# KDL-umass/CausalGPSLC.jl

Hardware: AMD Instinct MI355X
Metric: posterior samples/sec (kernel+chol+predict) at N=4096; SATE rel-err vs CPU (higher is better)
Workload: dtype f64; 1 GPU; Synthetic N=4096 D=8 nU=2, unit A (Gram build + potrf + alpha + MeanITE + SATE mean/var), L=1 level(s), 1024 posterior samples per GPU per step; levels=1, mean_ite=True

## Files before the change

### causalgpslc.jl_amd/csrc/back_block.h

```cpp
#pragma once
#include "gpslc_internal.h"

__device__ __forceinline__ void tile_tv32(const double* __restrict__ t, const double* v ,
                                          int wave, int lane, double out[32]) {
    const double v0 = v[lane], v1 = v[lane + 64];
    double p[32];
#pragma unroll
    for (int cc = 0; cc < 32; ++cc) {
        const double* col = t + (wave * 32 + cc) * GP_TS;
        p[cc] = col[lane] * v0 + col[lane + 64] * v1;
    }
#pragma unroll
    for (int cc = 0; cc < 32; ++cc) {
        double x = p[cc];
#pragma unroll
        for (int o = 32; o >= 1; o >>= 1) x += __shfl_xor(x, o, 64);
        out[cc] = x;
    }
}

__device__ __forceinline__ void tile_tv16_issue(const double* __restrict__ t, int wave, int half, int lane, double (&raw)[32]) {
#pragma unroll
    for (int cc = 0; cc < 16; ++cc) {
        const double* col = t + (wave * 32 + half * 16 + cc) * GP_TS;
        raw[cc] = __builtin_nontemporal_load(col + lane);
        raw[16 + cc] = __builtin_nontemporal_load(col + lane + 64);
    }
}
__device__ __forceinline__ double tile_tv16_finish(const double (&raw)[32], const double* v , int lane) {
    const double v0 = v[lane], v1 = v[lane + 64];
    double p[16], q8[8], q4[4], q2[2];
#pragma unroll
    for (int cc = 0; cc < 16; ++cc) p[cc] = raw[cc] * v0 + raw[16 + cc] * v1;
    const bool b5 = (lane & 32) != 0, b4 = (lane & 16) != 0, b3 = (lane & 8) != 0, b2 = (lane & 4) != 0;
#pragma unroll
    for (int j = 0; j < 8; ++j) {
        const double send = b5 ? p[j] : p[8 + j], keep = b5 ? p[8 + j] : p[j];
        q8[j] = keep + __shfl_xor(send, 32, 64);
    }
#pragma unroll
    for (int j = 0; j < 4; ++j) {
        const double send = b4 ? q8[j] : q8[4 + j], keep = b4 ? q8[4 + j] : q8[j];
        q4[j] = keep + __shfl_xor(send, 16, 64);
    }
#pragma unroll
    for (int j = 0; j < 2; ++j) {
        const double send = b3 ? q4[j] : q4[2 + j], keep = b3 ? q4[2 + j] : q4[j];
        q2[j] = keep + __shfl_xor(send, 8, 64);
    }
    const double send = b2 ? q2[0] : q2[1], keep = b2 ? q2[1] : q2[0];
    double x = keep + __shfl_xor(send, 4, 64);
    x += __shfl_xor(x, 2, 64);
    x += __shfl_xor(x, 1, 64);
    return x;
}

__device__ __forceinline__ void back_task_body(const TRef& M, const TRef& F, const int b, const int nt, double* __restrict__ alpha_out,
                                               double* lds, const int tid) {
    double* z = lds;
    double* al = lds + nt * GP_TS;
    const int lane = tid & 63;
    const int wave = __builtin_amdgcn_readfirstlane(tid >> 6);
    const int col = wave * 32 + (lane >> 2);
    const bool writer = (lane & 3) == 0;
    double ra[32], rb[32];
    tile_tv16_issue(tref_tile(F, b, 0, nt - 1), wave, 0, lane, ra);
    tile_tv16_issue(tref_tile(F, b, 0, nt - 1), wave, 1, lane, rb);
    for (int e = tid; e < nt * GP_TS; e += 256) z[e] = tref_tile(M, b, nt, e >> 7)[(e & 127) * GP_TS];
    __syncthreads();
    for (int i = nt - 1; i >= 0; --i) {
        {
            const double* nxt = i > 0 ? tref_tile(M, b, i, i - 1) : nullptr;
            const double m0 = tile_tv16_finish(ra, z + i * GP_TS, lane);
            if (nxt) tile_tv16_issue(nxt, wave, 0, lane, ra);
            const double m1 = tile_tv16_finish(rb, z + i * GP_TS, lane);
            if (nxt) tile_tv16_issue(nxt, wave, 1, lane, rb);
            if (writer) {
                al[i * GP_TS + col] = m0;
                al[i * GP_TS + col + 16] = m1;
                alpha_out[i * GP_TS + col] = m0;
                alpha_out[i * GP_TS + col + 16] = m1;
            }
        }
        __syncthreads();
        for (int k = i - 1; k >= 0; --k) {
            const double* nxt = k > 0 ? tref_tile(M, b, i, k - 1) : tref_tile(F, b, 0, i - 1);
            const double m0 = tile_tv16_finish(ra, al + i * GP_TS, lane);
            tile_tv16_issue(nxt, wave, 0, lane, ra);
            const double m1 = tile_tv16_finish(rb, al + i * GP_TS, lane);
            tile_tv16_issue(nxt, wave, 1, lane, rb);
            if (writer) {
                z[k * GP_TS + col] -= m0;
                z[k * GP_TS + col + 16] -= m1;
            }
        }
        __syncthreads();
    }
}
```

### causalgpslc.jl_amd/csrc/gpslc_internal.h

```cpp
#pragma once
#include <hip/hip_runtime.h>
#include <stdint.h>

#define GP_TS 128
#define GP_TSQ (GP_TS * GP_TS)

typedef double d4 __attribute__((ext_vector_type(4)));
typedef double d2 __attribute__((ext_vector_type(2)));

#define MAXF 32

#include <atomic>
#include <cstdlib>
struct DeviceOnce {
    std::atomic<unsigned long long> mask{0};
};
inline void lds_opt_in(DeviceOnce& o, const void* fn, int bytes) {
    int dev = 0;
    (void)hipGetDevice(&dev);
    const unsigned long long bit = 1ull << (dev & 63);
    if (o.mask.load(std::memory_order_acquire) & bit) return;
    (void)hipFuncSetAttribute(fn, hipFuncAttributeMaxDynamicSharedMemorySize, bytes);
    o.mask.fetch_or(bit, std::memory_order_release);
}
inline int device_cus() {
    static std::atomic<int> cus[64];
    int dev = 0;
    (void)hipGetDevice(&dev);
    int v = cus[dev & 63].load(std::memory_order_relaxed);
    if (v == 0) {
        v = 256;
        (void)hipDeviceGetAttribute(&v, hipDeviceAttributeMultiprocessorCount, dev);
        cus[dev & 63].store(v, std::memory_order_relaxed);
    }
    return v;
}
inline int diag_env(const char* name, int dflt) {
#ifdef GPSLC_DIAG
    const char* e = getenv(name);
    return e ? atoi(e) : dflt;
#else
    (void)name;
    return dflt;
#endif
}

struct TRef {
    double* base;
    long long bstride;
    int kind;
    int ro, co;
    int ld;
    int bdiv;
};

__host__ __device__ inline long long tref_index(const TRef& t, int i, int j) {
    long long ii = (long long)i + t.ro, jj = (long long)j + t.co;
    return t.kind == 0 ? ii * (ii + 1) / 2 + jj : ii * (long long)t.ld + jj;
}
__host__ __device__ inline double* tref_tile(const TRef& t, long long b, int i, int j) {
    if (t.bdiv > 1) b /= t.bdiv;
    return t.base + b * t.bstride + tref_index(t, i, j) * (long long)GP_TSQ;
}

struct GemmArgs {
    TRef A, B, C;
    int shape;
    int i0, j0;
    int mi, mj;
    int k0, k1;
    int accumulate;
    int nbatch;
    int ntiles;
    int short_row0;
    int short_rows;
    int sym;
    int fuse;
    TRef F;
    int fk;
    int skip_gdiag;
    int* info;
    int info_base;
    int* queue;
    const unsigned short* order;
    int diag_skip;
    unsigned long long* dbg;
};

struct SampleParams {
    const double* U;
    const double* uyLS;
    const double* xyLS;
    const double* tyLS;
    const double* yScale;
    const double* yNoise;
    long long u_sstride;
};

struct SampleGrid {
    const double* X;
    const double* T;
    SampleParams p;
    long long s0;
    int n, nX, nU, nt;
    __host__ __device__ const double* column(long long s, int f) const {
        return f < nU ? p.U + s * p.u_sstride + (long long)f * n : X + (long long)(f - nU) * n;
    }
    __host__ __device__ double lengthscale(long long s, int f) const {
        return f < nU ? p.uyLS[s * nU + f] : p.xyLS[s * nX + (f - nU)];
    }
};

struct GramArgs : SampleGrid {
    TRef M;
    double* part;
    int with_sums;
    int f32;
    int binary_t;
    unsigned long long* dbg;
};

#include "task_list.h"
struct PotrfTaskArgs {
    GemmArgs g;
    const unsigned* list;
    int* sync;
    int* timeout;
    int nt;
    double* alpha;
    int fence_mode;
    unsigned long long* dbg;
};
void launch_potrf_tasks(const PotrfTaskArgs& a, long long ntasks, int mt, hipStream_t st);

void launch_tile_gemm(const GemmArgs& g, hipStream_t st);
void launch_syrk_diag(const GemmArgs& g, int carry_aug, hipStream_t st);
void launch_diag_update_potrf(const GemmArgs& g, int carry_aug, hipStream_t st);
void launch_diag(const TRef& M, int k, double* inv, long long inv_bstride, int* info,
                 int info_base, int nbatch, hipStream_t st);
void launch_gram(const GramArgs& g, int nbatch, hipStream_t st);
void launch_diag_robust(const TRef& M, int k, int* info, int info_base, int nbatch, hipStream_t st);
void launch_trsm_robust(const TRef& X, const TRef& L, int k, int i0, int count, int nbatch, hipStream_t st);
void launch_fold_pair_info(const int* pair_info, int* info, int gs, int lc, hipStream_t st);

struct RhsArgs {
    const double* T; const double* Y; const double* tyLS; const double* doT;
    long long y_sstride;
    long long s0; int n, nt, naug, L; int with_sums;
    const double* part; double* bsum; double* ksum; double* sumdelta;
    TRef M;
    int live_rows;
    const double* doT_base;
    const double* W; int G;
    const double* bw; const double* kw; double* wnorm2;
};
void launch_rhs(const RhsArgs& r, int nbatch, hipStream_t st);

struct WsumArgs : SampleGrid {
    int G;
    const double* W;
    double* bw; double* kw;
    int with_k;
    int binary_t;
};
void launch_wsum(const WsumArgs& a, int nbatch, hipStream_t st);

struct EpiArgs {
    TRef M; int n, nt, naug, L; long long s0; long long S;
    const double* sumdelta; double pred_noise;
    double* meanSATE; double* varSATE;
    double* logdet; double* quad;
    int from_rows;
    const double* wnorm2; int wL;
};
void launch_epilogue(const EpiArgs& e, int nbatch, hipStream_t st);

struct BackArgs {
    TRef M; const double* inv; long long inv_bstride; int nt; int naug;
    double* zwork;
};
void launch_backsolve(const BackArgs& a, int nbatch, hipStream_t st);

struct IteMeanArgs : SampleGrid {
    long long S;
    int L; const double* doT;
    const double* alpha;
    const double* Y;
    long long y_sstride;
    const double* yNoise;
    double* meanITE;
    long long si, ss, sl;
    int f32;
    const double* doT_base;
};
void launch_ite_mean(const IteMeanArgs& a, int nbatch, hipStream_t st);

struct VecArgs : SampleGrid {
    int L;
    const double* doT;
    TRef M; double* part; double* sumdelta;
    const double* alpha; const double* Y; long long y_sstride;
    double* meanITE; long long si, ss, sl;
};
void launch_vec_sums(const VecArgs& a, int nbatch, hipStream_t st);
void launch_vec_mean(const VecArgs& a, int nbatch, hipStream_t st);

void launch_rbf_log(const double* X1, const double* X2, long long n, int d, const double* ls,
                    int ls_len, double* out, hipStream_t st);
void launch_process_cov(const double* in, long long n, double scale, double noise, double* out,
                        hipStream_t st);

struct DtArgs : SampleGrid {
    const double* doT;
    int l0, lc;
    int vec;
// ... 80 lines not shown
```

### causalgpslc.jl_amd/csrc/k_tilegemm.hip

```cpp
#include "gpslc_internal.h"
#include "diag_block.h"
#include "back_block.h"

#ifdef GPSLC_DIAG
#define GP_DBG_ON(g) ((g).dbg != nullptr)
#define GP_DIAG_SKIP(g) ((g).diag_skip)
#define GP_FENCE_MODE(a) ((a).fence_mode & 1)
#define GP_TASK_PRIO(a) (((a).fence_mode >> 4) & 3)
#define GP_TASK_WITHHOLD(a, b, is_diag, k) ((((a).fence_mode >> 6) & 1) && (b) == 0 && (is_diag) && (k) == 1)
#else
#define GP_DBG_ON(g) false
#define GP_DIAG_SKIP(g) 0
#define GP_FENCE_MODE(a) 0
#define GP_TASK_PRIO(a) 3
#define GP_TASK_WITHHOLD(a, b, is_diag, k) false
#endif

#define KLOOP_BARRIER asm volatile("s_waitcnt lgkmcnt(0)\n\ts_barrier" ::: "memory")
#define MFMA_PRIO_UP __builtin_amdgcn_s_setprio(1)
#define MFMA_PRIO_DOWN __builtin_amdgcn_s_setprio(0)

#define KS 16
#define LROW 144
#define OPER_LDS (KS * LROW)
// ... 140 lines not shown
                    xb[u] = *reinterpret_cast<const d2*>(pb + (tid + 256 * u) * 2);
                }
            };
            auto lstore = [&](int buf, const d2 (&xa)[4], const d2 (&xb)[4]) {
#pragma unroll
                for (int u = 0; u < 4; ++u) {
                    *reinterpret_cast<d2*>(lA + buf * OPER_LDS + loff[u]) = xa[u];
                    *reinterpret_cast<d2*>(lB + buf * OPER_LDS + loff[u]) = xb[u];
                }
            };
            auto compute = [&](int buf, int s) {
                const double* pa = lA + buf * OPER_LDS + frow_a;
                const double* pb = lB + buf * OPER_LDS + frow_b;
                const int nlo = ACC ? 0 : min(4, max(0, (s & 7) - 4 * wc));
                constexpr bool PIPE = ACC && DIAG == 0;
                double afn[4], bfn[4];
                if (PIPE) {
#pragma unroll
                    for (int m = 0; m < 4; ++m) afn[m] = pa[16 * m];
#pragma unroll
                    for (int n = 0; n < 4; ++n) bfn[n] = pb[16 * n];
                }
#pragma unroll
                for (int ks = 0; ks < KS / 4; ++ks) {
                    double af[4], bf[4];
                    if (PIPE) {
#pragma unroll
                        for (int m = 0; m < 4; ++m) { af[m] = afn[m]; bf[m] = bfn[m]; }
                        if (ks + 1 < KS / 4) {
#pragma unroll
                            for (int m = 0; m < 4; ++m) afn[m] = pa[(ks + 1) * 4 * LROW + 16 * m];
#pragma unroll
                            for (int n = 0; n < 4; ++n) bfn[n] = pb[(ks + 1) * 4 * LROW + 16 * n];
                        }
                    } else {
#pragma unroll
                        for (int m = 0; m < 4; ++m) af[m] = pa[ks * 4 * LROW + 16 * m];
#pragma unroll
                        for (int n = 0; n < 4; ++n) bf[n] = pb[ks * 4 * LROW + 16 * n];
                    }
                    if (mlive == 4 && nlo == 0) {
#pragma unroll
                        for (int m = 0; m < 4; ++m)
#pragma unroll
                            for (int n = 0; n < 4; ++n)
                                acc[m][n] = mfma_step<ACC>(bf[n], af[m], acc[m][n]);
                    } else {
#pragma unroll
                        for (int m = 0; m < 4; ++m)
                            if (m < mlive) {
#pragma unroll
                                for (int n = 0; n < 4; ++n)
                                    if (n >= nlo) acc[m][n] = mfma_step<ACC>(bf[n], af[m], acc[m][n]);
                            }
                    }
                }
            };

            auto compute_p = [&](int buf, int s) {
                const int sl = s & 7;
                if (sl > 7 - pw) return;
                const bool use0 = sl <= pw;
                const double* pa = lA + buf * OPER_LDS + (lane >> 4) * LROW + (lane & 15);
                const double* pb = lB + buf * OPER_LDS + (lane >> 4) * LROW + (lane & 15);
#pragma unroll
                for (int ks = 0; ks < KS / 4; ++ks) {
                    const double b0 = pb[ks * 4 * LROW + 16 * pw];
                    const double b1 = pb[ks * 4 * LROW + 16 * (7 - pw)];
                    double af[8];
#pragma unroll
                    for (int m = 0; m < 8; ++m) af[m] = pa[ks * 4 * LROW + 16 * m];
#pragma unroll
                    for (int m = 0; m < 8; ++m)
                        if (m < prow) {
                            if (use0) acc[m >> 1][2 * (m & 1)] = mfma_step<0>(b0, af[m], acc[m >> 1][2 * (m & 1)]);
                            acc[m >> 1][2 * (m & 1) + 1] = mfma_step<0>(b1, af[m], acc[m >> 1][2 * (m & 1) + 1]);
                        }
                }
            };

            gload(0, ra, rb);
            lstore(0, ra, rb);
            gload(1, ra, rb);
            __syncthreads();
            if (GP_DBG_ON(g)) st1 = __builtin_amdgcn_s_memtime();
            if (DIAG == 0) {
                for (int s = 0; s < nslab; s += 2) {
                    if (s + 2 < nslab) gload(s + 2, ra2, rb2);
                    MFMA_PRIO_UP;
                    if (ACC) compute(0, s); else compute_p(0, s);
                    MFMA_PRIO_DOWN;
                    lstore(1, ra, rb);
                    KLOOP_BARRIER;
                    if (s + 3 < nslab) gload(s + 3, ra, rb);
                    MFMA_PRIO_UP;
                    if (ACC) compute(1, s + 1); else compute_p(1, s + 1);
                    MFMA_PRIO_DOWN;
                    if (s + 2 < nslab) lstore(0, ra2, rb2);
                    KLOOP_BARRIER;
                }
            } else {
                for (int s = 0; s < nslab; s += 2) {
                    compute(0, s);
                    if (DIAG == 1) lstore(1, ra, rb);
                    __syncthreads();
                    compute(1, s + 1);
                    if (DIAG == 1) lstore(0, ra, rb);
                    __syncthreads();
                }
            }
        }
        if (GP_DBG_ON(g)) st2 = __builtin_amdgcn_s_memtime();

        {
        if (!ACC) {
            double* __restrict__ Cp = Ct + ((lane >> 4) * GP_TS + (lane & 15));
#pragma unroll
            for (int m = 0; m < 8; ++m)
                if (m < prow) {
#pragma unroll
                    for (int v = 0; v < 4; ++v) {
                        Cp[(16 * pw + 4 * v) * GP_TS + 16 * m] = acc[m >> 1][2 * (m & 1)][v];
                        Cp[(16 * (7 - pw) + 4 * v) * GP_TS + 16 * m] = acc[m >> 1][2 * (m & 1) + 1][v];
                    }
                }
        } else {
            int soff = ccol * GP_TS + crow;
            asm volatile("" : "+v"(soff));
            double* __restrict__ Cs = Ct + soff;
#pragma unroll
            for (int n = 0; n < 4; ++n)
#pragma unroll
                for (int v = 0; v < 4; ++v)
#pragma unroll
                    for (int m = 0; m < 4; ++m)
                        Cs[(16 * n + 4 * v) * GP_TS + 16 * m] = acc[m][n][v];
        }
        }
        if (GP_DBG_ON(g)) {
            asm volatile("s_waitcnt vmcnt(0)" ::: "memory");
            const unsigned long long st3 = __builtin_amdgcn_s_memtime();
            if (tid == 0) {
                unsigned long long* d = g.dbg + (size_t)item * 8;
                d[0] = st0; d[1] = st1; d[2] = st2; d[3] = st3;
                d[4] = __builtin_amdgcn_s_getreg((31 << 11) | 4);
                d[5] = __builtin_amdgcn_s_getreg((31 << 11) | 20);
                d[6] = __builtin_amdgcn_s_memrealtime();
                d[7] = blockIdx.x;
            }
        }
    });
}

typedef const __attribute__((address_space(1))) char* gcptr;
__device__ __forceinline__ gcptr wave_uniform(const void* p) {
    const unsigned long long x = (unsigned long long)p;
    const unsigned lo = __builtin_amdgcn_readfirstlane((unsigned)x);
    const unsigned hi = __builtin_amdgcn_readfirstlane((unsigned)(x >> 32));
    return (gcptr)(((unsigned long long)hi << 32) | lo);
}
typedef unsigned u4 __attribute__((ext_vector_type(4)));
template <bool WT>
__device__ __forceinline__ void strip_store2(__amdgpu_buffer_rsrc_t rs, double* tile_lane, int lane_bytes, int col_doubles, d2 v) {
    if (WT) __builtin_amdgcn_raw_buffer_store_b128(__builtin_bit_cast(u4, v), rs, lane_bytes + col_doubles * 8, 0,  16);
    else __builtin_nontemporal_store(v, reinterpret_cast<d2*>(tile_lane + col_doubles));
}

template <int WD, bool AUGEP = false, bool WT = false>
__device__ __forceinline__ void strip_item(const GemmArgs& g, const int b, const int ti, const int tj, const bool no_update,
                                           const int nslab, double* lB, const int tid, const int lane,
                                           const int wave, const int li, const int lg, const int frow_b,
                                           const int (&loff)[4], const long long item, const bool with_aug = false) {
    double* __restrict__ Ct = tref_tile(g.C, b, ti, tj);
    const bool live = !(g.short_rows > 0 && ti >= g.short_row0 && 32 * wave >= g.short_rows);
    unsigned long long st0 = 0, st1 = 0, st2 = 0;
    if (GP_DBG_ON(g)) st0 = __builtin_amdgcn_s_memtime();
    const int lane_off = lg * GP_TS + 32 * wave + 2 * li;

    d4 acc[2][8];
    if (live) {
        const double* __restrict__ Cl = Ct + lane_off;
#pragma unroll
        for (int n = 0; n < 8; ++n)
#pragma unroll
            for (int v = 0; v < 4; ++v) {
                const d2 c = __builtin_nontemporal_load(reinterpret_cast<const d2*>(Cl + (16 * n + 4 * v) * GP_TS));
                acc[0][n][v] = c[0];
                acc[1][n][v] = c[1];
            }
    }

    if (nslab > 0 && !no_update) {
        constexpr int SLAB = KS * GP_TS * 8;
        const int nsl = __builtin_amdgcn_readfirstlane(nslab);
        const __amdgpu_buffer_rsrc_t rA = __builtin_amdgcn_make_buffer_rsrc(
            (void*)(unsigned long long)wave_uniform(tref_tile(g.A, b, ti, g.k0)), 0, nsl * SLAB, 0x00020000);
        const __amdgpu_buffer_rsrc_t rB = __builtin_amdgcn_make_buffer_rsrc(
            (void*)(unsigned long long)wave_uniform(tref_tile(g.B, b, tj, g.k0)), 0, nsl * SLAB, 0x00020000);
        int voa[4], vob[4];
#pragma unroll
        for (int u = 0; u < 4; ++u) {
            voa[u] = (4 * u * GP_TS + lane_off) * 8;
            vob[u] = (tid + 256 * u) * 16;
        }
        const std::true_type yes;
        const std::false_type no;
        auto kloop = [&](auto lv) {
            constexpr bool LIVE = decltype(lv)::value;
            d2 rb[4], rb2[4];
            d2 a0[4], a1[4];
            auto bload1 = [&](int so, int u) { return __builtin_bit_cast(d2, __builtin_amdgcn_raw_buffer_load_b128(rB, vob[u], so, 0)); };
            auto bload = [&](int so, d2 (&xb)[4]) {
#pragma unroll
                for (int u = 0; u < 4; ++u) xb[u] = bload1(so, u);
            };
            auto aload = [&](int so, int ks) {
                return __builtin_bit_cast(d2, __builtin_amdgcn_raw_buffer_load_b128(rA, voa[ks], so,  2));
            };
            auto lstore = [&](int buf, const d2 (&xb)[4]) {
#pragma unroll
                for (int u = 0; u < 4; ++u) *reinterpret_cast<d2*>(lB + buf * OPER_LDS + loff[u]) = xb[u];
            };
            auto slab = [&](auto pf, int buf, d2 (&aa)[4], int so, d2 (&lb)[4], auto ws, int wbuf,
                            const d2 (&wb)[4]) {
                constexpr bool PF = decltype(pf)::value;
                constexpr bool WS = decltype(ws)::value;
                const double* pb = lB + buf * OPER_LDS + frow_b;
#pragma unroll
                for (int ks = 0; ks < KS / 4; ++ks) {
                    if (LIVE) {
                        double bf[8];
#pragma unroll
                        for (int n = 0; n < 8; ++n) bf[n] = pb[ks * 4 * LROW + 16 * n];
                        const d2 a = aa[ks];
#pragma unroll
                        for (int n = 0; n < 8; ++n)
#pragma unroll
                            for (int m = 0; m < 2; ++m) acc[m][n] = mfma_step<1>(bf[n], a[m], acc[m][n]);
                        if (PF) aa[ks] = aload(so, ks);
                    }
                    if (PF) lb[ks] = bload1(so, ks);
                    if (WS) *reinterpret_cast<d2*>(lB + wbuf * OPER_LDS + loff[ks]) = wb[ks];
                }
            };
            bload(0, rb);
            if (LIVE) {
#pragma unroll
                for (int ks = 0; ks < 4; ++ks) a0[ks] = aload(0, ks);
#pragma unroll
                for (int ks = 0; ks < 4; ++ks) a1[ks] = aload(SLAB, ks);
            }
            lstore(0, rb);
            bload(SLAB, rb);
            KLOOP_BARRIER;
            if (GP_DBG_ON(g)) st1 = __builtin_amdgcn_s_memtime();
            int so = 2 * SLAB;
            for (int s = 0; s + 2 < nsl; s += 2) {
                slab(yes, 0, a0, so, rb2, yes, 1, rb);
                KLOOP_BARRIER;
                slab(yes, 1, a1, so + SLAB, rb, yes, 0, rb2);
                KLOOP_BARRIER;
                so += 2 * SLAB;
            }
            slab(no, 0, a0, 0, rb2, yes, 1, rb);
            KLOOP_BARRIER;
            slab(no, 1, a1, 0, rb, no, 0, rb2);
            KLOOP_BARRIER;
        };
        if (live) kloop(yes); else kloop(no);
    }
    if (GP_DBG_ON(g)) st2 = __builtin_amdgcn_s_memtime();

    if (live) {
        const double* __restrict__ Wl = tref_tile(g.F, b, 0, g.fk) + (lg * GP_TS + li);
        double* __restrict__ Co = Ct + lane_off;
        const __amdgpu_buffer_rsrc_t crs = __builtin_amdgcn_make_buffer_rsrc((void*)(unsigned long long)wave_uniform(Ct), 0, GP_TSQ * 8, 0x00020000);
        double wn[WD];
        int pc = 0, pn = 0, pv = 0;
#pragma unroll
        for (int q = 0; q < WD; ++q) {
            wn[q] = Wl[(16 * pn + 4 * pv) * GP_TS + 16 * pc];
            if (++pv == 4) { pv = 0; if (++pn > pc) { pn = 0; ++pc; } }
        }
        int q = 0;
#pragma unroll
        for (int nc = 0; nc < 8; ++nc) {
            d4 st[2];
            st[0] = (d4){0.0, 0.0, 0.0, 0.0};
            st[1] = (d4){0.0, 0.0, 0.0, 0.0};
#pragma unroll
            for (int n = 0; n < 8; ++n)
                if (n <= nc) {
#pragma unroll
                    for (int v = 0; v < 4; ++v) {
                        const double w = wn[q % WD];
                        if (pc < 8) {
                            wn[q % WD] = Wl[(16 * pn + 4 * pv) * GP_TS + 16 * pc];
                            if (++pv == 4) { pv = 0; if (++pn > pc) { pn = 0; ++pc; } }
                        }
                        ++q;
                        st[0] = mfma_step<0>(w, acc[0][n][v], st[0]);
                        st[1] = mfma_step<0>(w, acc[1][n][v], st[1]);
                    }
                }
#pragma unroll
            for (int v = 0; v < 4; ++v)
                strip_store2<WT>(crs, Co, lane_off * 8, (16 * nc + 4 * v) * GP_TS, (d2){st[0][v], st[1][v]});
        }
    }
    if (AUGEP && with_aug) {
        const int mrows = (g.short_rows + 15) >> 4;
        double* __restrict__ Cg = tref_tile(g.C, b, g.short_row0, tj) + (lg * GP_TS + li);
        const double* __restrict__ Wl = tref_tile(g.F, b, 0, g.fk) + (lg * GP_TS + li);
// ... 101 lines not shown
        for (int m = 0; m < MT; ++m)
#pragma unroll
            for (int v = 0; v < 4; ++v) {
                ag[m][0][v] = Cg[(16 * W + 4 * v) * GP_TS + 16 * m];
                ag[m][1][v] = Cg[(16 * (7 - W) + 4 * v) * GP_TS + 16 * m];
            }
    }
    if (nslab <= 0) return;
    int loff[4];
    stage_offsets(tid, loff);
    const bool glive = MT > 0 && tid < 128 * MT;
    const int gcol = tid / (8 * (MT > 0 ? MT : 1)), grp = tid % (8 * (MT > 0 ? MT : 1));
    d2 rs[SYRK_PF][4], rgs[MT > 0 ? SYRK_PF : 1];
    auto gload = [&](int s, int set) {
        const int kk = g.k0 + (s >> 3);
        const double* pa = tref_tile(g.A, b, t, kk) + (s & 7) * (KS * GP_TS);
#pragma unroll
        for (int u = 0; u < 4; ++u) rs[set][u] = *reinterpret_cast<const d2*>(pa + (tid + 256 * u) * 2);
        if (MT > 0 && glive) {
            const double* pg = tref_tile(g.A, b, g.short_row0, kk) + (s & 7) * (KS * GP_TS);
            rgs[MT > 0 ? set : 0] = *reinterpret_cast<const d2*>(pg + gcol * GP_TS + 2 * grp);
        }
    };
    auto lstore = [&](int buf, int set) {
#pragma unroll
        for (int u = 0; u < 4; ++u) *reinterpret_cast<d2*>(lA + buf * OPER_LDS + loff[u]) = rs[set][u];
        if (MT > 0 && glive)
            *reinterpret_cast<d2*>(lG + buf * OPER_LDS + gcol * LROW + 2 * grp) = rgs[MT > 0 ? set : 0];
    };
    auto compute = [&](int buf) {
        const double* pa = lA + buf * OPER_LDS + fbase;
        const double* pg = lG + buf * OPER_LDS + fbase;
#pragma unroll
        for (int ks = 0; ks < KS / 4; ++ks) {
            double bf[8 - W];
#pragma unroll
            for (int cb = 0; cb < 8 - W; ++cb) bf[cb] = pa[ks * 4 * LROW + 16 * cb];
            const double r0 = pa[ks * 4 * LROW + 16 * W];
            const double r1 = pa[ks * 4 * LROW + 16 * (7 - W)];
#pragma unroll
            for (int cb = 0; cb <= W; ++cb) a0c[cb] = mfma_step<1>(bf[cb], r0, a0c[cb]);
#pragma unroll
            for (int cb = 0; cb < 8 - W; ++cb) a1c[cb] = mfma_step<1>(bf[cb], r1, a1c[cb]);
            if (MT > 0) {
#pragma unroll
                for (int m = 0; m < MT; ++m) {
                    const double gf = pg[ks * 4 * LROW + 16 * m];
                    ag[m][0] = mfma_step<1>(bf[W], gf, ag[m][0]);
                    ag[m][1] = mfma_step<1>(bf[7 - W], gf, ag[m][1]);
                }
            }
        }
    };
#pragma unroll
    for (int u = 0; u < SYRK_PF; ++u) gload(u, u);
    lstore(0, 0);
    KLOOP_BARRIER;
    for (int s = 0; s < nslab; s += SYRK_PF) {
#pragma unroll
        for (int u = 0; u < SYRK_PF; ++u) {
            if (s + u + SYRK_PF < nslab) gload(s + u + SYRK_PF, u);
            compute(u & 1);
            if (s + u + 1 < nslab) lstore((u + 1) & 1, (u + 1) % SYRK_PF);
            KLOOP_BARRIER;
        }
    }
}

template <int W, int MT, bool WT = false>
__device__ __forceinline__ void syrk_chain_wave(const GemmArgs& g, const int b, const int td, const int kd1, double* smem,
                                                const int tid, const int lane) {
    d4 a0c[W + 1], a1c[8 - W], ag[MT > 0 ? MT : 1][2];
    diag_tile_update<W, MT>(g, b, td, (kd1 - g.k0) * (GP_TS / KS), smem, tid, lane, a0c, a1c, ag);
    const int li = lane & 15, lg = lane >> 4;
#pragma unroll
    for (int cb = 0; cb <= W; ++cb)
#pragma unroll
        for (int v = 0; v < 4; ++v) smem[(((W * (W + 1)) / 2 + cb) << 8) + (lg + 4 * v) * 16 + li] = a0c[cb][v];
#pragma unroll
    for (int cb = 0; cb < 8 - W; ++cb)
#pragma unroll
        for (int v = 0; v < 4; ++v) smem[((((7 - W) * (8 - W)) / 2 + cb) << 8) + (lg + 4 * v) * 16 + li] = a1c[cb][v];
    if (MT > 0) {
        double* __restrict__ Cg = tref_tile(g.C, b, g.short_row0, td) + (lg * GP_TS + li);
#pragma unroll
        for (int m = 0; m < MT; ++m)
#pragma unroll
            for (int v = 0; v < 4; ++v) {
                out_store<WT>(Cg + (16 * W + 4 * v) * GP_TS + 16 * m, ag[m][0][v]);
                out_store<WT>(Cg + (16 * (7 - W) + 4 * v) * GP_TS + 16 * m, ag[m][1][v]);
            }
    }
}

template <int MT>
__global__ __launch_bounds__(256, 2) void diag_update_potrf_kernel(GemmArgs g) {
    extern __shared__ __attribute__((aligned(16))) double smem[];
    const int tid = threadIdx.x, lane = tid & 63;
    const int b = blockIdx.x;
    const int td = g.i0;
    switch (__builtin_amdgcn_readfirstlane(tid >> 6)) {
        case 0: syrk_chain_wave<0, MT>(g, b, td, g.k1, smem, tid, lane); break;
        case 1: syrk_chain_wave<1, MT>(g, b, td, g.k1, smem, tid, lane); break;
        case 2: syrk_chain_wave<2, MT>(g, b, td, g.k1, smem, tid, lane); break;
        default: syrk_chain_wave<3, MT>(g, b, td, g.k1, smem, tid, lane); break;
    }
    diag_potrf_inv_la_body(smem, tref_tile(g.C, b, td, td), tref_tile(g.F, b, 0, td), g.info + b, g.info_base + GP_TS * td,
                           tid, true);
}

static unsigned persistent_grid(long long work) {
    const int slots = 2 * device_cus();
    return (unsigned)(work < slots ? work : slots);
}
template <class F>
static void dispatch_mt(int mt, F&& launch) {
    if (mt == 0) launch(std::integral_constant<int, 0>());
    else if (mt == 1) launch(std::integral_constant<int, 1>());
    else launch(std::integral_constant<int, 2>());
}

template <int MT>
static void launch_diag_update_potrf_t(const GemmArgs& g, hipStream_t st) {
    static DeviceOnce once;
    constexpr int bytes = DIAG3_LDS_BYTES > GEMM_LDS_BYTES ? DIAG3_LDS_BYTES : GEMM_LDS_BYTES;
    lds_opt_in(once, (const void*)diag_update_potrf_kernel<MT>, bytes);
    hipLaunchKernelGGL(diag_update_potrf_kernel<MT>, dim3(g.nbatch), dim3(256), bytes, st, g);
}

void launch_diag_update_potrf(const GemmArgs& g, int carry_aug, hipStream_t st) {
    if (g.nbatch <= 0) return;
    dispatch_mt(carry_aug ? (g.short_rows + 15) / 16 : 0,
                [&](auto mt) { launch_diag_update_potrf_t<decltype(mt)::value>(g, st); });
}

#define TASK_POLL_LIMIT (1 << 20)

__device__ __forceinline__ int task_progress_load(const int* p) {
    return __hip_atomic_load(p, __ATOMIC_RELAXED, __HIP_MEMORY_SCOPE_AGENT);
}
__device__ __forceinline__ void task_wait(const int* p, int need, int* tmo) {
    if (task_progress_load(p) >= need) return;
    for (int spins = 0;; ++spins) {
        __builtin_amdgcn_s_sleep(8);
        if (task_progress_load(p) >= need) return;
        if ((spins & 63) == 63 && task_progress_load(tmo) != 0) return;
        if (spins > TASK_POLL_LIMIT) {
            __hip_atomic_store(tmo, 1, __ATOMIC_RELAXED, __HIP_MEMORY_SCOPE_AGENT);
            return;
        }
    }
}

__device__ __forceinline__ unsigned task_fetch(const PotrfTaskArgs& a, int& q, int& visited) {
    while (visited < 8) {
        const int len = (int)a.list[8 + q];
        const int t = len > 0 ? atomicAdd(&a.sync[q], 1) : len;
        if (t < len) return a.list[TASK_LIST_HDR + a.list[q] + t];
        q = (q + 1) & 7;
        ++visited;
    }
    return TASK_NONE;
}

template <int MT, bool WT>
__global__ __launch_bounds__(256, 2) void potrf_tasks_kernel(PotrfTaskArgs a) {
    extern __shared__ __attribute__((aligned(16))) double smem[];
    __shared__ unsigned s_desc, s_next;
    __shared__ int s_q, s_visited;
    __shared__ unsigned long long s_ready;
    if (threadIdx.x == 0) {
        int q = (int)(__builtin_amdgcn_s_getreg((31 << 11) | 20) & 7);
        int visited = 0;
        s_next = task_fetch(a, q, visited);
        s_q = q; s_visited = visited;
    }
    for (;;) {
        int tid = threadIdx.x;
        asm volatile("" : "+v"(tid));
        unsigned long long stf = 0;
        if (GP_DBG_ON(a)) stf = __builtin_amdgcn_s_memtime();
        if (tid == 0) {
            int* const tmo = a.timeout;
            const unsigned d = s_next;
            if (d != TASK_NONE) {
                const int nt = a.nt;
                const int b = TASK_B(d), k = TASK_K(d), i = TASK_I(d), rows = TASK_ROWS(d);
                const int* prog = a.sync + TASK_SYNC_HDR + (long long)b * TASK_SYNC_STRIDE;
                if ((d >> 30) == 3) {
                    task_wait(prog, nt, tmo);
                    task_wait(prog + 1 + nt, nt, tmo);
                } else if ((d >> 30) & 1) {
                    if (k > 0) {
                        task_wait(prog + 1 + k, k, tmo);
                        if (MT > 0) task_wait(prog + 1 + nt, k, tmo);
                        if (rows > 1) task_wait(prog + 2 + k, k, tmo);
                    }
                } else {
                    task_wait(prog, k + 1, tmo);
                    if ((i < nt || MT == 0) && k > 0)
                        for (int r = 0; r < rows; ++r) task_wait(prog + 1 + i + r, k, tmo);
                }
                if (GP_DBG_ON(a)) s_ready = __builtin_amdgcn_s_memtime();
                __builtin_amdgcn_fence(__ATOMIC_ACQUIRE, "agent");
                asm volatile("s_waitcnt vmcnt(0)" ::: "memory");
            }
            s_desc = d;
        }
        __syncthreads();
        const unsigned d = s_desc;
        if (d == TASK_NONE) break;
        const int b = TASK_B(d), k = TASK_K(d), i = TASK_I(d), rows = TASK_ROWS(d);
        const bool is_back = (d >> 30) == 3;
        const bool is_diag = (d >> 30) == 1;
        const bool with_aug = (d >> 30) == 2;
        unsigned long long st0 = 0, st1 = 0;
        if (GP_DBG_ON(a)) st0 = __builtin_amdgcn_s_memtime();
        int tnext = 0, qn = 0, lenn = 0;
        if (tid == 0) {
            qn = s_q;
            lenn = s_visited < 8 ? (int)a.list[8 + qn] : 0;
            tnext = lenn > 0 ? atomicAdd(&a.sync[qn], 1) : 0;
        }
        const int lane = tid & 63;
        const int wave = __builtin_amdgcn_readfirstlane(tid >> 6);
        if (is_back) {
            back_task_body(a.g.C, a.g.F, b, a.nt, a.alpha + (long long)b * a.nt * GP_TS, smem, tid);
        } else if (is_diag) {
            if (GP_TASK_PRIO(a) == 3) __builtin_amdgcn_s_setprio(3);
            else if (GP_TASK_PRIO(a) == 1) __builtin_amdgcn_s_setprio(1);
            double* tile = tref_tile(a.g.C, b, k, k);
            double* invt = tref_tile(a.g.F, b, 0, k);
            if (k == 0) {
                diag_potrf_inv_la_body<WT>(smem, tile, invt, a.g.info + b, a.g.info_base, tid, false);
            } else {
                switch (wave) {
                    case 0: syrk_chain_wave<0, MT, WT>(a.g, b, k, k, smem, tid, lane); break;
                    case 1: syrk_chain_wave<1, MT, WT>(a.g, b, k, k, smem, tid, lane); break;
                    case 2: syrk_chain_wave<2, MT, WT>(a.g, b, k, k, smem, tid, lane); break;
                    default: syrk_chain_wave<3, MT, WT>(a.g, b, k, k, smem, tid, lane); break;
                }
                diag_potrf_inv_la_body<WT>(smem, tile, invt, a.g.info + b, a.g.info_base + GP_TS * k, tid, true);
            }
            __builtin_amdgcn_s_setprio(0);
        }
        const bool diag_then_strip = is_diag && rows > 1;
        if (diag_then_strip) {
            asm volatile("s_waitcnt vmcnt(0)" ::: "memory");
            __syncthreads();
        }
        if ((!is_diag && !is_back) || diag_then_strip) {
            const int li = lane & 15, lg = lane >> 4;
            int loff[4];
            stage_offsets(tid, loff);
            GemmArgs gl = a.g;
            gl.k1 = k;
            gl.fk = k;
            if (diag_then_strip)
                strip_item<FUSE_WD, (MT > 0), WT>(gl, b, k + 1, k, false, 8 * k, smem, tid, lane, wave, li, lg, lg * LROW + li, loff, 0,
                                              true);
            else
                for (int r = 0; r < rows; ++r)
                    strip_item<FUSE_WD, (MT > 0), WT>(gl, b, i + r, k, MT > 0 && i >= a.nt, 8 * k, smem, tid, lane, wave, li, lg,
                                                  lg * LROW + li, loff, 0, with_aug && r == 0);
        }
        asm volatile("s_waitcnt vmcnt(0)" ::: "memory");
        __syncthreads();
        if (GP_DBG_ON(a)) st1 = __builtin_amdgcn_s_memtime();
        if (tid == 0) {
            unsigned dn = TASK_NONE;
            const bool hit = tnext < lenn;
            if (hit) dn = a.list[TASK_LIST_HDR + a.list[qn] + tnext];
            int* prog = a.sync + TASK_SYNC_HDR + (long long)b * TASK_SYNC_STRIDE;
            if (!is_back && !GP_TASK_WITHHOLD(a, b, is_diag, k)) {
                if (GP_FENCE_MODE(a) == 0 && !WT) __builtin_amdgcn_fence(__ATOMIC_RELEASE, "agent");
                asm volatile("s_waitcnt vmcnt(0)" ::: "memory");
                if (is_diag) {
                    __hip_atomic_store(prog, k + 1, __ATOMIC_RELAXED, __HIP_MEMORY_SCOPE_AGENT);
                    if (diag_then_strip) {
                        __hip_atomic_store(prog + 2 + k, k + 1, __ATOMIC_RELAXED, __HIP_MEMORY_SCOPE_AGENT);
                        if (MT > 0) __hip_atomic_store(prog + 1 + a.nt, k + 1, __ATOMIC_RELAXED, __HIP_MEMORY_SCOPE_AGENT);
                    }
                } else
                    for (int r = 0; r < rows; ++r)
                        __hip_atomic_store(prog + 1 + i + r, k + 1, __ATOMIC_RELAXED, __HIP_MEMORY_SCOPE_AGENT);
                if (with_aug) __hip_atomic_store(prog + 1 + a.nt, k + 1, __ATOMIC_RELAXED, __HIP_MEMORY_SCOPE_AGENT);
            }
            if (!hit) {
                int q = qn, visited = s_visited;
                if (visited < 8) { q = (q + 1) & 7; ++visited; }
                dn = task_fetch(a, q, visited);
                s_q = q; s_visited = visited;
            }
            s_next = dn;
            if (GP_DBG_ON(a)) {
                unsigned long long* dd = a.dbg + 8 * (size_t)atomicAdd(a.sync + 9, 1);
                dd[0] = stf; dd[1] = st0; dd[2] = st1; dd[3] = __builtin_amdgcn_s_memtime(); dd[4] = d; dd[5] = blockIdx.x;
                dd[6] = s_ready; dd[7] = __builtin_amdgcn_s_getreg((31 << 11) | 20);
            }
        }
    }
}

template <int MT, bool WT>
static void launch_potrf_tasks_t(const PotrfTaskArgs& a, unsigned grid, hipStream_t st) {
    static DeviceOnce once;
    constexpr int bytes = DIAG3_LDS_BYTES > GEMM_LDS_BYTES ? DIAG3_LDS_BYTES : GEMM_LDS_BYTES;
    lds_opt_in(once, (const void*)potrf_tasks_kernel<MT, WT>, bytes);
    hipLaunchKernelGGL((potrf_tasks_kernel<MT, WT>), dim3(grid), dim3(256), bytes, st, a);
}

void launch_potrf_tasks(const PotrfTaskArgs& a, long long ntasks, int mt, hipStream_t st) {
    if (ntasks <= 0) return;
    const unsigned grid = persistent_grid(ntasks);
#ifdef GPSLC_DIAG
    if (a.fence_mode & 2) {
        dispatch_mt(mt, [&](auto m) { launch_potrf_tasks_t<decltype(m)::value, false>(a, grid, st); });
        return;
    }
#endif
    dispatch_mt(mt, [&](auto m) { launch_potrf_tasks_t<decltype(m)::value, true>(a, grid, st); });
}

#define DG_LDS_BYTES(MT) ((2 * OPER_LDS + ((MT) > 0 ? 2 * OPER_LDS : 0)) * 8)

template <int W, int MT>
__device__ __forceinline__ void syrk_diag_wave(const GemmArgs& g, double* smem, int tid, int lane) {
    const XcdSplit x = xcd_split((long long)g.mi * g.nbatch);
    const int nslab = (g.k1 - g.k0) * (GP_TS / KS);
    const int li = lane & 15, lg = lane >> 4;
    for (long long it = x.local; it < x.xc; it += x.gx) {
        const long long item = x.x0 + it;
        const int b = (int)(item / g.mi);
        const int ti = g.i0 + (int)(item - (long long)b * g.mi);
        d4 a0c[W + 1], a1c[8 - W], ag[MT > 0 ? MT : 1][2];
        diag_tile_update<W, MT>(g, b, ti, nslab, smem, tid, lane, a0c, a1c, ag);
        double* __restrict__ Cd = tref_tile(g.C, b, ti, ti) + (lg * GP_TS + li);
#pragma unroll
        for (int cb = 0; cb <= W; ++cb)
#pragma unroll
            for (int v = 0; v < 4; ++v) Cd[(16 * cb + 4 * v) * GP_TS + 16 * W] = a0c[cb][v];
#pragma unroll
        for (int cb = 0; cb < 8 - W; ++cb)
#pragma unroll
            for (int v = 0; v < 4; ++v) Cd[(16 * cb + 4 * v) * GP_TS + 16 * (7 - W)] = a1c[cb][v];
        if (MT > 0) {
            double* __restrict__ Cg = tref_tile(g.C, b, g.short_row0, ti) + (lg * GP_TS + li);
#pragma unroll
            for (int m = 0; m < MT; ++m)
#pragma unroll
                for (int v = 0; v < 4; ++v) {
                    Cg[(16 * W + 4 * v) * GP_TS + 16 * m] = ag[m][0][v];
                    Cg[(16 * (7 - W) + 4 * v) * GP_TS + 16 * m] = ag[m][1][v];
                }
        }
    }
}

template <int MT>
__global__ __launch_bounds__(256, 2) void tile_syrk_diag_kernel(GemmArgs g) {
    extern __shared__ __attribute__((aligned(16))) double smem[];
    const int tid = threadIdx.x, lane = tid & 63;
    switch (__builtin_amdgcn_readfirstlane(tid >> 6)) {
        case 0: syrk_diag_wave<0, MT>(g, smem, tid, lane); break;
        case 1: syrk_diag_wave<1, MT>(g, smem, tid, lane); break;
        case 2: syrk_diag_wave<2, MT>(g, smem, tid, lane); break;
        default: syrk_diag_wave<3, MT>(g, smem, tid, lane); break;
    }
}

template <int MT>
static void launch_syrk_diag_t(const GemmArgs& g, unsigned grid, hipStream_t st) {
    static DeviceOnce once;
    lds_opt_in(once, (const void*)tile_syrk_diag_kernel<MT>, DG_LDS_BYTES(MT));
    hipLaunchKernelGGL(tile_syrk_diag_kernel<MT>, dim3(grid), dim3(256), DG_LDS_BYTES(MT), st, g);
}

void launch_syrk_diag(const GemmArgs& g, int carry_aug, hipStream_t st) {
    if (g.mi <= 0 || g.nbatch <= 0 || g.k1 <= g.k0) return;
    const unsigned grid = persistent_grid((long long)g.mi * g.nbatch);
    dispatch_mt(carry_aug ? (g.short_rows + 15) / 16 : 0,
                [&](auto mt) { launch_syrk_diag_t<decltype(mt)::value>(g, grid, st); });
}

template <int ACC, int DIAG>
static void launch_one(const GemmArgs& g, unsigned grid, hipStream_t st) {
    static DeviceOnce once;
    lds_opt_in(once, (const void*)tile_gemm_nt_kernel<ACC, DIAG>, GEMM_LDS_BYTES);
    hipLaunchKernelGGL((tile_gemm_nt_kernel<ACC, DIAG>), dim3(grid), dim3(256), GEMM_LDS_BYTES, st, g);
}

void launch_tile_gemm(const GemmArgs& g, hipStream_t st) {
    if (g.ntiles <= 0 || g.nbatch <= 0) return;
    const unsigned grid = persistent_grid((long long)g.ntiles * g.nbatch);
#ifdef GPSLC_DIAG
    if (g.diag_skip == 1) {
        if (g.accumulate) launch_one<1, 1>(g, grid, st); else launch_one<0, 1>(g, grid, st);
        return;
    }
    if (g.diag_skip == 2) {
        if (g.accumulate) launch_one<1, 2>(g, grid, st); else launch_one<0, 2>(g, grid, st);
        return;
    }
#endif
    if (g.fuse && g.accumulate) {
        static DeviceOnce once;
        lds_opt_in(once, (const void*)tile_fused_strip_kernel<FUSE_WD>, STRIP_LDS_BYTES);
        hipLaunchKernelGGL((tile_fused_strip_kernel<FUSE_WD>), dim3(grid), dim3(256), STRIP_LDS_BYTES, st, g);
    } else {
        if (g.accumulate) launch_one<1, 0>(g, grid, st); else launch_one<0, 0>(g, grid, st);
    }
}
```

Before: 2440 posterior samples/s.

## Use buffer loads and DPP/permlane reductions in back-solve; streamline task fetch and waits

The back-substitution tile matvec now loads through buffer resources with scalar offsets and replaces shfl_xor reductions with permlane32/16 swaps and DPP row/quad ops, which should cut LDS-crossbar traffic and VGPR address math. The vector operands are read from LDS once per outer iteration instead of inside every finish. The persistent task scheduler caches queue offset and length in shared memory and prefetches the next descriptor before the barrier. It also polls all dependency counters at once before spinning, which shortens critical-path latency between tasks. The change relies on gfx950-specific permlane-swap builtins and on more complex queue-state encoding.

```diff
diff --git a/causalgpslc.jl_amd/csrc/back_block.h b/causalgpslc.jl_amd/csrc/back_block.h
--- a/causalgpslc.jl_amd/csrc/back_block.h
+++ b/causalgpslc.jl_amd/csrc/back_block.h
@@ -19,62 +19,95 @@
     }
 }
 
-__device__ __forceinline__ void tile_tv16_issue(const double* __restrict__ t, int wave, int half, int lane, double (&raw)[32]) {
+typedef unsigned u2 __attribute__((ext_vector_type(2)));
+__device__ __forceinline__ __amdgpu_buffer_rsrc_t tile_rsrc(const double* t) {
+    return __builtin_amdgcn_make_buffer_rsrc((void*)(unsigned long long)wave_uniform(t), 0, GP_TSQ * 8, 0x00020000);
+}
+__device__ __forceinline__ void tile_tv16_issue(const __amdgpu_buffer_rsrc_t rs, int wave, int half, int lane8, double (&raw)[32]) {
+    const int s0 = (wave * 32 + half * 16) * (GP_TS * 8);
 #pragma unroll
     for (int cc = 0; cc < 16; ++cc) {
-        const double* col = t + (wave * 32 + half * 16 + cc) * GP_TS;
-        raw[cc] = __builtin_nontemporal_load(col + lane);
-        raw[16 + cc] = __builtin_nontemporal_load(col + lane + 64);
+        const int so = s0 + (cc >> 2) * (4 * GP_TS * 8), io = (cc & 3) * (GP_TS * 8);
+        raw[cc] = __builtin_bit_cast(double, __builtin_amdgcn_raw_buffer_load_b64(rs, lane8 + io, so,  2));
+        raw[16 + cc] = __builtin_bit_cast(double, __builtin_amdgcn_raw_buffer_load_b64(rs, lane8 + io + 64 * 8, so,  2));
     }
 }
-__device__ __forceinline__ double tile_tv16_finish(const double (&raw)[32], const double* v , int lane) {
-    const double v0 = v[lane], v1 = v[lane + 64];
+__device__ __forceinline__ double swap_add32(double a, double b) {
+    const u2 ua = __builtin_bit_cast(u2, a), ub = __builtin_bit_cast(u2, b);
+    const auto lo = __builtin_amdgcn_permlane32_swap(ua.x, ub.x, false, false);
+    const auto hi = __builtin_amdgcn_permlane32_swap(ua.y, ub.y, false, false);
+    const u2 ra = {lo[0], hi[0]}, rb = {lo[1], hi[1]};
+    return __builtin_bit_cast(double, ra) + __builtin_bit_cast(double, rb);
+}
+__device__ __forceinline__ double swap_add16(double a, double b) {
+    const u2 ua = __builtin_bit_cast(u2, a), ub = __builtin_bit_cast(u2, b);
+    const auto lo = __builtin_amdgcn_permlane16_swap(ua.x, ub.x, false, false);
+    const auto hi = __builtin_amdgcn_permlane16_swap(ua.y, ub.y, false, false);
+    const u2 ra = {lo[0], hi[0]}, rb = {lo[1], hi[1]};
+    return __builtin_bit_cast(double, ra) + __builtin_bit_cast(double, rb);
+}
+template <int O>
+__device__ __forceinline__ double swap_add_row(double a, double b) {
+    static_assert(O == 8 || O == 4, "row steps");
+    constexpr int HI = O == 8 ? 0xC : 0xA, LO = O == 8 ? 0x3 : 0x5;
+    constexpr int SHR = 0x110 + O, SHL = 0x100 + O;
+    const u2 ua = __builtin_bit_cast(u2, a), ub = __builtin_bit_cast(u2, b);
+    u2 ra, rb;
+    ra.x = __builtin_amdgcn_update_dpp(ua.x, ub.x, SHR, 0xF, HI, false);
+    ra.y = __builtin_amdgcn_update_dpp(ua.y, ub.y, SHR, 0xF, HI, false);
+    rb.x = __builtin_amdgcn_update_dpp(ub.x, ua.x, SHL, 0xF, LO, false);
+    rb.y = __builtin_amdgcn_update_dpp(ub.y, ua.y, SHL, 0xF, LO, false);
+    return __builtin_bit_cast(double, ra) + __builtin_bit_cast(double, rb);
+}
+template <int QP>
+__device__ __forceinline__ double quad_add(double x) {
+    const u2 ux = __builtin_bit_cast(u2, x);
+    u2 r;
+    r.x = __builtin_amdgcn_mov_dpp(ux.x, QP, 0xF, 0xF, false);
+    r.y = __builtin_amdgcn_mov_dpp(ux.y, QP, 0xF, 0xF, false);
+    return x + __builtin_bit_cast(double, r);
+}
+__device__ __forceinline__ double tile_tv16_finish(const double (&raw)[32], const double v0, const double v1) {
     double p[16], q8[8], q4[4], q2[2];
 #pragma unroll
     for (int cc = 0; cc < 16; ++cc) p[cc] = raw[cc] * v0 + raw[16 + cc] * v1;
-    const bool b5 = (lane & 32) != 0, b4 = (lane & 16) != 0, b3 = (lane & 8) != 0, b2 = (lane & 4) != 0;
 #pragma unroll
-    for (int j = 0; j < 8; ++j) {
-        const double send = b5 ? p[j] : p[8 + j], keep = b5 ? p[8 + j] : p[j];
-        q8[j] = keep + __shfl_xor(send, 32, 64);
-    }
+    for (int j = 0; j < 8; ++j) q8[j] = swap_add32(p[j], p[8 + j]);
 #pragma unroll
-    for (int j = 0; j < 4; ++j) {
-        const double send = b4 ? q8[j] : q8[4 + j], keep = b4 ? q8[4 + j] : q8[j];
-        q4[j] = keep + __shfl_xor(send, 16, 64);
-    }
+    for (int j = 0; j < 4; ++j) q4[j] = swap_add16(q8[j], q8[4 + j]);
 #pragma unroll
-    for (int j = 0; j < 2; ++j) {
-        const double send = b3 ? q4[j] : q4[2 + j], keep = b3 ? q4[2 + j] : q4[j];
-        q2[j] = keep + __shfl_xor(send, 8, 64);
-    }
-    const double send = b2 ? q2[0] : q2[1], keep = b2 ? q2[1] : q2[0];
-    double x = keep + __shfl_xor(send, 4, 64);
-    x += __shfl_xor(x, 2, 64);
-    x += __shfl_xor(x, 1, 64);
+    for (int j = 0; j < 2; ++j) q2[j] = swap_add_row<8>(q4[j], q4[2 + j]);
+    double x = swap_add_row<4>(q2[0], q2[1]);
+    x = quad_add<0x4E>(x);
+    x = quad_add<0xB1>(x);
     return x;
 }
 
-__device__ __forceinline__ void back_task_body(const TRef& M, const TRef& F, const int b, const int nt, double* __restrict__ alpha_out,
+__device__ __forceinline__ void back_task_body(const TRef& M, const TRef& F, const int b_, const int nt, double* __restrict__ alpha_out,
                                                double* lds, const int tid) {
     double* z = lds;
     double* al = lds + nt * GP_TS;
-    const int lane = tid & 63;
+    const int b = __builtin_amdgcn_readfirstlane(b_);
+    const int lane = tid & 63, lane8 = lane * 8;
     const int wave = __builtin_amdgcn_readfirstlane(tid >> 6);
     const int col = wave * 32 + (lane >> 2);
     const bool writer = (lane & 3) == 0;
     double ra[32], rb[32];
-    tile_tv16_issue(tref_tile(F, b, 0, nt - 1), wave, 0, lane, ra);
-    tile_tv16_issue(tref_tile(F, b, 0, nt - 1), wave, 1, lane, rb);
+    {
+        const __amdgpu_buffer_rsrc_t rs = tile_rsrc(tref_tile(F, b, 0, nt - 1));
+        tile_tv16_issue(rs, wave, 0, lane8, ra);
+        tile_tv16_issue(rs, wave, 1, lane8, rb);
+    }
     for (int e = tid; e < nt * GP_TS; e += 256) z[e] = tref_tile(M, b, nt, e >> 7)[(e & 127) * GP_TS];
     __syncthreads();
     for (int i = nt - 1; i >= 0; --i) {
         {
-            const double* nxt = i > 0 ? tref_tile(M, b, i, i - 1) : nullptr;
-            const double m0 = tile_tv16_finish(ra, z + i * GP_TS, lane);
-            if (nxt) tile_tv16_issue(nxt, wave, 0, lane, ra);
-            const double m1 = tile_tv16_finish(rb, z + i * GP_TS, lane);
-            if (nxt) tile_tv16_issue(nxt, wave, 1, lane, rb);
+            const double v0 = z[i * GP_TS + lane], v1 = z[i * GP_TS + lane + 64];
+            const __amdgpu_buffer_rsrc_t rs = tile_rsrc(tref_tile(M, b, i, i > 0 ? i - 1 : 0));
+            const double m0 = tile_tv16_finish(ra, v0, v1);
+            if (i > 0) tile_tv16_issue(rs, wave, 0, lane8, ra);
+            const double m1 = tile_tv16_finish(rb, v0, v1);
+            if (i > 0) tile_tv16_issue(rs, wave, 1, lane8, rb);
             if (writer) {
                 al[i * GP_TS + col] = m0;
                 al[i * GP_TS + col + 16] = m1;
@@ -83,12 +116,13 @@
             }
         }
         __syncthreads();
+        const double v0 = al[i * GP_TS + lane], v1 = al[i * GP_TS + lane + 64];
         for (int k = i - 1; k >= 0; --k) {
-            const double* nxt = k > 0 ? tref_tile(M, b, i, k - 1) : tref_tile(F, b, 0, i - 1);
-            const double m0 = tile_tv16_finish(ra, al + i * GP_TS, lane);
-            tile_tv16_issue(nxt, wave, 0, lane, ra);
-            const double m1 = tile_tv16_finish(rb, al + i * GP_TS, lane);
-            tile_tv16_issue(nxt, wave, 1, lane, rb);
+            const __amdgpu_buffer_rsrc_t rs = tile_rsrc(k > 0 ? tref_tile(M, b, i, k - 1) : tref_tile(F, b, 0, i - 1));
+            const double m0 = tile_tv16_finish(ra, v0, v1);
+            tile_tv16_issue(rs, wave, 0, lane8, ra);
+            const double m1 = tile_tv16_finish(rb, v0, v1);
+            tile_tv16_issue(rs, wave, 1, lane8, rb);
             if (writer) {
                 z[k * GP_TS + col] -= m0;
                 z[k * GP_TS + col + 16] -= m1;
diff --git a/causalgpslc.jl_amd/csrc/gpslc_internal.h b/causalgpslc.jl_amd/csrc/gpslc_internal.h
--- a/causalgpslc.jl_amd/csrc/gpslc_internal.h
+++ b/causalgpslc.jl_amd/csrc/gpslc_internal.h
@@ -61,6 +61,14 @@
 __host__ __device__ inline double* tref_tile(const TRef& t, long long b, int i, int j) {
     if (t.bdiv > 1) b /= t.bdiv;
     return t.base + b * t.bstride + tref_index(t, i, j) * (long long)GP_TSQ;
+}
+
+typedef const __attribute__((address_space(1))) char* gcptr;
+__device__ __forceinline__ gcptr wave_uniform(const void* p) {
+    const unsigned long long x = (unsigned long long)p;
+    const unsigned lo = __builtin_amdgcn_readfirstlane((unsigned)x);
+    const unsigned hi = __builtin_amdgcn_readfirstlane((unsigned)(x >> 32));
+    return (gcptr)(((unsigned long long)hi << 32) | lo);
 }
 
 struct GemmArgs {
diff --git a/causalgpslc.jl_amd/csrc/k_tilegemm.hip b/causalgpslc.jl_amd/csrc/k_tilegemm.hip
--- a/causalgpslc.jl_amd/csrc/k_tilegemm.hip
+++ b/causalgpslc.jl_amd/csrc/k_tilegemm.hip
@@ -316,13 +316,6 @@
     });
 }
 
-typedef const __attribute__((address_space(1))) char* gcptr;
-__device__ __forceinline__ gcptr wave_uniform(const void* p) {
-    const unsigned long long x = (unsigned long long)p;
-    const unsigned lo = __builtin_amdgcn_readfirstlane((unsigned)x);
-    const unsigned hi = __builtin_amdgcn_readfirstlane((unsigned)(x >> 32));
-    return (gcptr)(((unsigned long long)hi << 32) | lo);
-}
 typedef unsigned u4 __attribute__((ext_vector_type(4)));
 template <bool WT>
 __device__ __forceinline__ void strip_store2(__amdgpu_buffer_rsrc_t rs, double* tile_lane, int lane_bytes, int col_doubles, d2 v) {
@@ -730,11 +723,19 @@
     }
 }
 
-__device__ __forceinline__ unsigned task_fetch(const PotrfTaskArgs& a, int& q, int& visited) {
+__device__ __forceinline__ void task_wait3(const int* p0, int n0, const int* p1, int n1, const int* p2, int n2, int* tmo) {
+    const int v0 = task_progress_load(p0), v1 = task_progress_load(p1), v2 = task_progress_load(p2);
+    if (v0 < n0) task_wait(p0, n0, tmo);
+    if (v1 < n1) task_wait(p1, n1, tmo);
+    if (v2 < n2) task_wait(p2, n2, tmo);
+}
+
+__device__ __forceinline__ unsigned task_fetch(const PotrfTaskArgs& a, int& q, int& visited, int& off, int& len) {
     while (visited < 8) {
-        const int len = (int)a.list[8 + q];
+        len = (int)a.list[8 + q];
+        off = (int)a.list[q];
         const int t = len > 0 ? atomicAdd(&a.sync[q], 1) : len;
-        if (t < len) return a.list[TASK_LIST_HDR + a.list[q] + t];
+        if (t < len) return a.list[TASK_LIST_HDR + off + t];
         q = (q + 1) & 7;
         ++visited;
     }
@@ -744,14 +745,14 @@
 template <int MT, bool WT>
 __global__ __launch_bounds__(256, 2) void potrf_tasks_kernel(PotrfTaskArgs a) {
     extern __shared__ __attribute__((aligned(16))) double smem[];
-    __shared__ unsigned s_desc, s_next;
-    __shared__ int s_q, s_visited;
+    __shared__ unsigned s_desc;
+    __shared__ int s_qv, s_qoff, s_qlen;
     __shared__ unsigned long long s_ready;
     if (threadIdx.x == 0) {
         int q = (int)(__builtin_amdgcn_s_getreg((31 << 11) | 20) & 7);
-        int visited = 0;
-        s_next = task_fetch(a, q, visited);
-        s_q = q; s_visited = visited;
+        int visited = 0, off = 0, len = 0;
+        s_desc = task_fetch(a, q, visited, off, len);
+        s_qv = q | (visited << 3); s_qoff = off; s_qlen = len;
     }
     for (;;) {
         int tid = threadIdx.x;
@@ -760,30 +761,28 @@
         if (GP_DBG_ON(a)) stf = __builtin_amdgcn_s_memtime();
         if (tid == 0) {
             int* const tmo = a.timeout;
-            const unsigned d = s_next;
+            const unsigned d = s_desc;
             if (d != TASK_NONE) {
                 const int nt = a.nt;
                 const int b = TASK_B(d), k = TASK_K(d), i = TASK_I(d), rows = TASK_ROWS(d);
                 const int* prog = a.sync + TASK_SYNC_HDR + (long long)b * TASK_SYNC_STRIDE;
+                constexpr int NO_WAIT = -2147483647 - 1;
                 if ((d >> 30) == 3) {
-                    task_wait(prog, nt, tmo);
-                    task_wait(prog + 1 + nt, nt, tmo);
+                    task_wait3(prog, nt, prog + 1 + nt, nt, prog, NO_WAIT, tmo);
                 } else if ((d >> 30) & 1) {
-                    if (k > 0) {
-                        task_wait(prog + 1 + k, k, tmo);
-                        if (MT > 0) task_wait(prog + 1 + nt, k, tmo);
-                        if (rows > 1) task_wait(prog + 2 + k, k, tmo);
-                    }
+                    if (k > 0)
+                        task_wait3(prog + 1 + k, k, prog + 1 + nt, MT > 0 ? k : NO_WAIT, prog + 2 + k, rows > 1 ? k : NO_WAIT, tmo);
                 } else {
-                    task_wait(prog, k + 1, tmo);
-                    if ((i < nt || MT == 0) && k > 0)
-                        for (int r = 0; r < rows; ++r) task_wait(prog + 1 + i + r, k, tmo);
+                    const bool tile_rows = (i < nt || MT == 0) && k > 0;
+                    task_wait3(prog, k + 1, prog + 1 + i, tile_rows ? k : NO_WAIT, prog + 1 + i + (rows > 1 ? 1 : 0),
+                               tile_rows && rows > 1 ? k : NO_WAIT, tmo);
+                    if (tile_rows)
+                        for (int r = 2; r < rows; ++r) task_wait(prog + 1 + i + r, k, tmo);
                 }
                 if (GP_DBG_ON(a)) s_ready = __builtin_amdgcn_s_memtime();
                 __builtin_amdgcn_fence(__ATOMIC_ACQUIRE, "agent");
                 asm volatile("s_waitcnt vmcnt(0)" ::: "memory");
             }
-            s_desc = d;
         }
         __syncthreads();
         const unsigned d = s_desc;
@@ -794,12 +793,8 @@
         const bool with_aug = (d >> 30) == 2;
         unsigned long long st0 = 0, st1 = 0;
         if (GP_DBG_ON(a)) st0 = __builtin_amdgcn_s_memtime();
-        int tnext = 0, qn = 0, lenn = 0;
-        if (tid == 0) {
-            qn = s_q;
-            lenn = s_visited < 8 ? (int)a.list[8 + qn] : 0;
-            tnext = lenn > 0 ? atomicAdd(&a.sync[qn], 1) : 0;
-        }
+        int tnext = 0;
+        if (tid == 0) tnext = atomicAdd(&a.sync[s_qv & 7], 1);
         const int lane = tid & 63;
         const int wave = __builtin_amdgcn_readfirstlane(tid >> 6);
         if (is_back) {
@@ -842,13 +837,13 @@
                     strip_item<FUSE_WD, (MT > 0), WT>(gl, b, i + r, k, MT > 0 && i >= a.nt, 8 * k, smem, tid, lane, wave, li, lg,
                                                   lg * LROW + li, loff, 0, with_aug && r == 0);
         }
+        unsigned dn = TASK_NONE;
+        if (tid == 0 && tnext < s_qlen) dn = a.list[TASK_LIST_HDR + s_qoff + tnext];
         asm volatile("s_waitcnt vmcnt(0)" ::: "memory");
         __syncthreads();
         if (GP_DBG_ON(a)) st1 = __builtin_amdgcn_s_memtime();
         if (tid == 0) {
-            unsigned dn = TASK_NONE;
-            const bool hit = tnext < lenn;
-            if (hit) dn = a.list[TASK_LIST_HDR + a.list[qn] + tnext];
+            const bool hit = dn != TASK_NONE;
             int* prog = a.sync + TASK_SYNC_HDR + (long long)b * TASK_SYNC_STRIDE;
             if (!is_back && !GP_TASK_WITHHOLD(a, b, is_diag, k)) {
                 if (GP_FENCE_MODE(a) == 0 && !WT) __builtin_amdgcn_fence(__ATOMIC_RELEASE, "agent");
@@ -865,12 +860,12 @@
                 if (with_aug) __hip_atomic_store(prog + 1 + a.nt, k + 1, __ATOMIC_RELAXED, __HIP_MEMORY_SCOPE_AGENT);
             }
             if (!hit) {
-                int q = qn, visited = s_visited;
+                int q = s_qv & 7, visited = s_qv >> 3, off = 0, len = 0;
                 if (visited < 8) { q = (q + 1) & 7; ++visited; }
-                dn = task_fetch(a, q, visited);
-                s_q = q; s_visited = visited;
-            }
-            s_next = dn;
+                dn = task_fetch(a, q, visited, off, len);
+                s_qv = q | (visited << 3); s_qoff = off; s_qlen = len;
+            }
+            s_desc = dn;
             if (GP_DBG_ON(a)) {
                 unsigned long long* dd = a.dbg + 8 * (size_t)atomicAdd(a.sync + 9, 1);
                 dd[0] = stf; dd[1] = st0; dd[2] = st1; dd[3] = __builtin_amdgcn_s_memtime(); dd[4] = d; dd[5] = blockIdx.x;
```

Result: no change. 2440 posterior samples/s (median of 3 runs) (-0.0%).
